# nexoedge/nexoedge

Measured on AMD Instinct MI355X. Metric: GiB/s RS(10,4) encode+decode, 1 MiB chunks, device-resident, higher is better.
Workload: dtype u8

## Files before the change

### nexoedge_amd/csrc/nxec_kernels.hip

```cpp
#include <hip/hip_runtime.h>

#include <algorithm>
#include <array>
#include <atomic>
#include <cstdio>
#include <cstdlib>
#include <cstring>
#include <utility>

#include "nxec_device.h"
#include "nxec_internal.h"
#include "nxec_scrub_rule.h"

namespace nxec {

namespace {

constexpr int kBlock = 1024;
constexpr int kMaxTemplK = 20;
constexpr int kLdsBytes = 160 * 1024;
constexpr int kPrefetchMaxK = 10;
constexpr int kPrefetchMaxKCopy = 8;
constexpr int kPermPrefetchMaxK = 4;
constexpr int kPermMaxK = 13;
// ... 122 lines not shown
template <int KD, int ROWS, int R>
struct ScrubBody {
  static constexpr int K = KD + ROWS;
  static constexpr int kLds = table_bytes(KD, R);
  static __device__ __forceinline__ void setup(const MulArgs &a, uint32_t *tab) {
    build_tables<R>(a.coef, KD, ROWS, tab);
  }
  const char *tlane;
  int32_t *status;
  __device__ ScrubBody(const uint32_t *tab, int32_t *st)
      : tlane(reinterpret_cast<const char *>(tab) + (threadIdx.x % R) * 4), status(st) {}
  __device__ __forceinline__ void operator()(const MulArgs &, uint32_t s, uint32_t, const u32x4 (&d)[K]) const {
    uint32_t acc[16];
    lookup_sources<KD, R>(tlane, d, acc);
    uint32_t o[4][4];
    rows_of(acc, o);
    uint32_t bad = 0;
#pragma unroll
    for (int r = 0; r < ROWS; r++)
      bad |= (o[r][0] ^ d[KD + r].x) | (o[r][1] ^ d[KD + r].y) | (o[r][2] ^ d[KD + r].z) | (o[r][3] ^ d[KD + r].w);
    const uint64_t hit = __ballot(bad != 0);
    if (hit != 0) {
      if (static_cast<int>(__lane_id()) == __ffsll(static_cast<unsigned long long>(hit)) - 1) scrub_flag(status, s);
    }
  }
};

__device__ __forceinline__ uint32_t perm_mul(const uint32_t *t, uint32_t nl, uint32_t nh, uint32_t ml, uint32_t mh) {
  const uint32_t l0 = __builtin_amdgcn_perm(t[1], t[0], nl), l1 = __builtin_amdgcn_perm(t[3], t[2], nl);
  const uint32_t h0 = __builtin_amdgcn_perm(t[5], t[4], nh), h1 = __builtin_amdgcn_perm(t[7], t[6], nh);
  return ((ml & l1) | (~ml & l0)) ^ ((mh & h1) | (~mh & h0));
}

template <int K, bool GATHER, bool COPY>
struct PermBody {
  static constexpr int kLds = K * 32;
  static __device__ __forceinline__ void setup(const MulArgs &a, uint32_t *tab) {
    uint8_t *tb = reinterpret_cast<uint8_t *>(tab);
    for (int i = threadIdx.x; i < K * 16; i += blockDim.x) {
      const int j = i >> 4, n = i & 15;
      const uint32_t c = a.coef[j];
      tb[32 * j + n] = static_cast<uint8_t>(gf_mul_dev(c, n));
      tb[32 * j + 16 + n] = static_cast<uint8_t>(gf_mul_dev(c, n << 4));
    }
  }
  const uint32_t *tab;
  __device__ explicit PermBody(const uint32_t *t) : tab(t) {}
  __device__ __forceinline__ void operator()(const MulArgs &a, uint32_t s, uint32_t vg, const u32x4 (&d)[K]) const {
    uint32_t z;
    asm volatile("s_mov_b32 %0, 0" : "=s"(z));
    const uint32_t *tt = tab + z;
    uint32_t o[4] = {0, 0, 0, 0};
#pragma unroll
    for (int j = 0; j < K; j++) {
      const uint32_t w[4] = {d[j].x, d[j].y, d[j].z, d[j].w};
#pragma unroll
      for (int q = 0; q < 4; q++) {
        const uint32_t x = w[q], x4 = x << 4;
        const uint32_t nl = x & 0x07070707u, nh = (x >> 4) & 0x07070707u;
        const uint32_t ml = __builtin_amdgcn_perm(x4, x4 << 8, 0x0B090A08u);
        const uint32_t mh = __builtin_amdgcn_perm(x, x << 8, 0x0B090A08u);
        o[q] ^= perm_mul(tt + 8 * j, nl, nh, ml, mh);
      }
    }
    st_stream(dst_row<GATHER>(a, s, 0) + static_cast<size_t>(vg) * 16, u32x4{o[0], o[1], o[2], o[3]});
    copy_through<K, COPY>(a, s, vg, d);
  }
};

__device__ uint32_t g_tile_queue[kQueueSlots * 32];

__device__ __forceinline__ uint32_t grab_async(uint32_t *q) {
  uint32_t g;
  asm volatile("global_atomic_add %0, %1, %2, off sc0" : "=&v"(g) : "v"(q), "v"(1u) : "memory");
  return g;
}
template <int N, int OFF>
__device__ __forceinline__ void publish(uint32_t ring_base, uint32_t g) {
  static_assert(N >= 0 && N < 64, "vmcnt is 6 bits");
  asm volatile("s_waitcnt vmcnt(%2)\n\tds_write_b32 %0, %1 offset:%3" ::"v"(ring_base), "v"(g), "n"(N), "n"(OFF)
               : "memory");
}

template <int K, bool PF, bool Q, bool QWAIT_K, class LoadF, class RunF>
__device__ __forceinline__ void tile_loop(const LoadF &load, const RunF &run, uint32_t ntiles, int32_t slot_arg,
                                          uint32_t T, uint32_t *ring) {
  if (Q && slot_arg >= 0) {
    uint32_t *q = g_tile_queue + static_cast<size_t>(slot_arg) * 32;
    if (threadIdx.x == 0) {
      ring[2] = atomicAdd(q, 1u);
      ring[3] = atomicAdd(q, 1u);
    }
    __syncthreads();
    auto run_start = [&](uint32_t r) -> uint32_t { return r * T; };
    uint32_t t = run_start(__builtin_amdgcn_readfirstlane(ring[2]));
    uint32_t nrun = run_start(__builtin_amdgcn_readfirstlane(ring[3]));
    uint32_t rend = t + T < ntiles ? t + T : ntiles;
    int slot = 0;
    uint32_t ring_base = static_cast<uint32_t>(reinterpret_cast<uintptr_t>(ring));
    asm volatile("" : "+v"(ring_base));
    auto ring_barrier = [] {
      __builtin_amdgcn_fence(__ATOMIC_RELEASE, "workgroup", "local");
      __builtin_amdgcn_s_barrier();
      __builtin_amdgcn_fence(__ATOMIC_ACQUIRE, "workgroup", "local");
    };
    auto step = [&](u32x4(&cur)[K], u32x4(&nxt)[K], bool pf) {
      const bool edge = t + 1 >= rend;
      const uint32_t tn = edge ? nrun : t + 1;
      uint32_t g = 0;
      if (edge && threadIdx.x == 0) g = grab_async(q);
      if (pf) {
        load(tn < ntiles ? tn : t, nxt);
        __builtin_amdgcn_sched_barrier(0);
      } else {
        load(t, cur);
        __builtin_amdgcn_sched_barrier(0);
      }
      run(t, cur);
      if (edge) {
        if (threadIdx.x == 0) {
          if (slot == 0) publish<QWAIT_K ? K : 0, 0>(ring_base, g);
          else publish<QWAIT_K ? K : 0, 4>(ring_base, g);
        }
        ring_barrier();
        const uint32_t nn = run_start(__builtin_amdgcn_readfirstlane(ring[slot]));
        slot ^= 1;
        rend = nrun + T < ntiles ? nrun + T : ntiles;
        nrun = nn;
      }
      t = tn;
      return t < ntiles;
    };
    if (t < ntiles) {
      if constexpr (PF) {
        u32x4 A[K], B[K];
        load(t, A);
        while (step(A, B, true) && step(B, A, true)) {
        }
      } else {
        bool more = true;
        while (more) {
          u32x4 d[K];
          more = step(d, d, false);
        }
      }
    }
    if (threadIdx.x == 0) {
      __threadfence();
      if (atomicAdd(q + 1, 1u) == gridDim.x - 1) {
        atomicExch(q, 0u);
        atomicExch(q + 1, 0u);
      }
    }
    return;
  }
  uint32_t t = __builtin_amdgcn_readfirstlane(
      static_cast<uint32_t>((static_cast<uint64_t>(blockIdx.x) * ntiles) / gridDim.x));
  const uint32_t tend = __builtin_amdgcn_readfirstlane(
      static_cast<uint32_t>((static_cast<uint64_t>(blockIdx.x + 1) * ntiles) / gridDim.x));
  if (t >= tend) return;
  if constexpr (PF) {
    u32x4 A[K], B[K];
    load(t, A);
    while (true) {
      const uint32_t tb = t + 1;
      load(tb < tend ? tb : t, B);
      __builtin_amdgcn_sched_barrier(0);
      run(t, A);
      if (tb >= tend) break;
      t = tb;
      const uint32_t ta = t + 1;
      load(ta < tend ? ta : t, A);
      __builtin_amdgcn_sched_barrier(0);
      run(t, B);
      if (ta >= tend) break;
      t = ta;
    }
  } else {
    for (; t < tend; t++) {
      u32x4 d[K];
      load(t, d);
      run(t, d);
    }
  }
}

template <int K, bool GATHER, bool FULL, bool PF, bool Q, class Body>
__device__ __forceinline__ void mul_tiles(const MulArgs &a, const Body &body, uint32_t *ring) {
  const uint32_t nvec = static_cast<uint32_t>(a.vec_count);
  const uint32_t tps = (nvec + kBlock - 1) / kBlock;
  const uint32_t ntiles = tps * static_cast<uint32_t>(a.nstripes);
  const uint32_t sg = a.stripe_group, ns = static_cast<uint32_t>(a.nstripes);
  auto load = [&](uint32_t t, u32x4(&d)[K]) { load_tile<K, GATHER, FULL>(a, tile_pos(t, tps, sg, ns), nvec, d); };
  auto run = [&](uint32_t t, const u32x4(&d)[K]) {
    const TilePos p = tile_pos(t, tps, sg, ns);
    if (FULL || p.v < nvec) body(a, p.s, static_cast<uint32_t>(a.vec_begin) + p.v, d);
  };
  tile_loop<K, PF, Q, FULL>(load, run, ntiles, a.queue_slot, a.tiles_per_grab, ring);
}

template <int K, int R, bool GATHER, bool COPY, bool FULL>
__global__ __launch_bounds__(kBlock) void k_mul_vec(const MulArgs a) {
  constexpr bool PF = vec_prefetch(K, COPY, FULL);
  constexpr bool Q = vec_queued(K, R);
  using Body = LdsBody<K, R, GATHER, COPY>;
  static_assert(Body::kLds + (Q ? kRingBytes : 0) == vec_lds(K, R), "tables, then the ring: what the launch asks for");
  extern __shared__ uint32_t tab[];
  Body::setup(a, tab);
  __syncthreads();
  mul_tiles<K, GATHER, FULL, PF, Q>(a, Body(tab), tab + Body::kLds / 4);
}

template <int K, bool GATHER, bool COPY, bool FULL>
__global__ __launch_bounds__(kBlock) void k_mul_perm(const MulArgs a) {
  constexpr bool PF = perm_prefetch(K);
  using Body = PermBody<K, GATHER, COPY>;
  static_assert(Body::kLds + kRingBytes == perm_lds(K), "tables, then the ring: what the launch asks for");
  extern __shared__ uint32_t tab[];
  Body::setup(a, tab);
  __syncthreads();
  mul_tiles<K, GATHER, FULL, PF, true>(a, Body(tab), tab + Body::kLds / 4);
}

struct RaggedArgs {
  const ListStripe *__restrict__ stripes;
  const uint32_t *__restrict__ tile_stripe;
  const uint32_t *__restrict__ stripe_tile0;
  uint32_t ntiles;
  int32_t k, rows, row0, queue_slot;
  uint32_t tiles_per_grab;
  uint8_t coef[kMaxRowsPerPass * (NXEC_MAX_K + 1)];
};

template <int K, int R>
__global__ __launch_bounds__(kBlock) void k_mul_ragged(const RaggedArgs a) {
  constexpr bool PF = ragged_prefetch(K);
  constexpr int kLds = table_bytes(K, R);
  static_assert(R == default_r(K) && kLds + kRingBytes == ragged_lds(K), "ragged kernels are queue-driven");
  extern __shared__ uint32_t tab[];
  build_tables<R>(a.coef, K, a.rows, tab);
  __syncthreads();
  const char *tl = reinterpret_cast<const char *>(tab) + (threadIdx.x % R) * 4;
  auto where = [&](uint32_t t, ListStripe &st, uint32_t &v) {
    const uint32_t s = a.tile_stripe[t];
    st = a.stripes[s];
    v = (t - a.stripe_tile0[s]) * kBlock + threadIdx.x;
  };
  auto load = [&](uint32_t t, u32x4(&d)[K]) {
    ListStripe st;
    uint32_t v;
    where(t, st, v);
    if (v * int64_t(16) < st.len) {
#pragma unroll
      for (int j = 0; j < K; j++) d[j] = ld_stream(st.src + j * st.src_cs + static_cast<size_t>(v) * 16);
    }
  };
  auto run = [&](uint32_t t, const u32x4(&d)[K]) {
    ListStripe st;
    uint32_t v;
    where(t, st, v);
    if (v * int64_t(16) < st.len) {
      uint32_t acc[16];
      lookup_sources<K, R>(tl, d, acc);
      uint8_t *row0 = st.dst + a.row0 * st.dst_cs;
      const int rows = a.rows;
      store_rows(acc, rows, [=](int r) { return row0 + r * st.dst_cs + static_cast<size_t>(v) * 16; });
    }
  };
  tile_loop<K, PF, true, true>(load, run, a.ntiles, a.queue_slot, a.tiles_per_grab, tab + kLds / 4);
}

struct MixedArgs {
  uint8_t *base;
  int64_t stripe_stride;
  const MixedSeg *__restrict__ segs;
  const uint32_t *__restrict__ order;
  const uint32_t *__restrict__ seg_of;
  uint32_t ntiles, tps, nvec;
  int32_t queue_slot;
  uint32_t tiles_per_grab;
};

constexpr int mixed_lds(int k) { return vec_lds(k, default_r(k)); }

template <class T>
__device__ __forceinline__ const __attribute__((address_space(4))) T *const_table(const T *p) {
  return (const __attribute__((address_space(4))) T *)(reinterpret_cast<uintptr_t>(p));
}

template <int K, int R>
__global__ __launch_bounds__(kBlock) void k_mul_mixed(const MixedArgs a) {
  constexpr bool PF = ragged_prefetch(K);
  constexpr int kLds = table_bytes(K, R);
  static_assert(R == default_r(K) && kLds + kRingBytes == mixed_lds(K), "mixed kernels are queue-driven");
  extern __shared__ uint32_t tab[];
  const char *tl = reinterpret_cast<const char *>(tab) + (threadIdx.x % R) * 4;
  uint32_t resident = ~0u;
  struct Where {
    uint32_t s, g, v;
  };
  auto where = [&](uint32_t t) -> Where {
    const uint32_t i = t / a.tps;
    return {static_cast<uint32_t>(__builtin_amdgcn_readfirstlane(const_table(a.order)[i])),
            static_cast<uint32_t>(__builtin_amdgcn_readfirstlane(const_table(a.seg_of)[i])),
            (t - i * a.tps) * kBlock + threadIdx.x};
  };
  auto load = [&](uint32_t t, u32x4(&d)[K]) {
    const Where w = where(t);
    if (w.v < a.nvec) {
      const auto *sg = const_table(a.segs) + w.g;
      const uint8_t *sb = a.base + static_cast<int64_t>(w.s) * a.stripe_stride;
      const uint32_t vo = w.v * 16u;
#pragma unroll
      for (int j = 0; j < K; j++) d[j] = ld_stream(sb + sg->src_off[j] + vo);
    }
  };
  auto run = [&](uint32_t t, const u32x4(&d)[K]) {
    const Where w = where(t);
    const auto *sg = const_table(a.segs) + w.g;
    const int rows = static_cast<int>(sg->rows);
    if (w.g != resident) {
      __builtin_amdgcn_fence(__ATOMIC_RELEASE, "workgroup", "local");
      __builtin_amdgcn_s_barrier();
      build_tables<R>(a.segs[w.g].coef, K, rows, tab);
      __builtin_amdgcn_fence(__ATOMIC_RELEASE, "workgroup", "local");
      __builtin_amdgcn_s_barrier();
      __builtin_amdgcn_fence(__ATOMIC_ACQUIRE, "workgroup", "local");
      resident = w.g;
    }
    if (w.v < a.nvec) {
      uint32_t acc[16];
      lookup_sources<K, R>(tl, d, acc);
      uint8_t *db = a.base + static_cast<int64_t>(w.s) * a.stripe_stride;
      const uint32_t vo = w.v * 16u;
      const uint32_t o0 = sg->dst_off[0], o1 = sg->dst_off[1], o2 = sg->dst_off[2], o3 = sg->dst_off[3];
      store_rows(acc, rows, [=](int r) { return db + (r == 0 ? o0 : r == 1 ? o1 : r == 2 ? o2 : o3) + vo; });
    }
  };
  tile_loop<K, PF, true, true>(load, run, a.ntiles, a.queue_slot, a.tiles_per_grab, tab + kLds / 4);
}

struct DecodeMixedArgs {
  const uint8_t *__restrict__ src;
  uint8_t *__restrict__ dst;
  int64_t src_stripe_stride, dst_stripe_stride;
  const DecodeSeg *__restrict__ segs;
  const uint32_t *__restrict__ order;
  const uint32_t *__restrict__ seg_of;
  uint32_t ntiles, tps, nvec;
  int32_t queue_slot;
  uint32_t tiles_per_grab;
};

constexpr int decode_mixed_lds(int k) { return vec_lds(k, default_r(k)); }

template <int K, int R>
__global__ __launch_bounds__(kBlock) void k_decode_mixed(const DecodeMixedArgs a) {
  constexpr bool PF = ragged_prefetch(K);
  constexpr int kLds = table_bytes(K, R);
  static_assert(K <= kMaxDecodeMixedK && R == default_r(K) && kLds + kRingBytes == decode_mixed_lds(K),
                "decode kernels are queue-driven");
  extern __shared__ uint32_t tab[];
  const char *tl = reinterpret_cast<const char *>(tab) + (threadIdx.x % R) * 4;
  uint32_t resident = ~0u;
  struct Where {
    uint32_t s, g, v;
  };
  auto where = [&](uint32_t t) -> Where {
    const uint32_t i = t / a.tps;
    return {static_cast<uint32_t>(__builtin_amdgcn_readfirstlane(const_table(a.order)[i])),
            static_cast<uint32_t>(__builtin_amdgcn_readfirstlane(const_table(a.seg_of)[i])),
            (t - i * a.tps) * kBlock + threadIdx.x};
  };
  auto load = [&](uint32_t t, u32x4(&d)[K]) {
    const Where w = where(t);
    if (w.v < a.nvec) {
      const auto *sg = const_table(a.segs) + w.g;
      const uint8_t *sb = a.src + static_cast<int64_t>(w.s) * a.src_stripe_stride;
      const uint32_t vo = w.v * 16u;
#pragma unroll
      for (int j = 0; j < K; j++) d[j] = ld_stream(sb + sg->src_off[j] + vo);
    }
  };
  auto run = [&](uint32_t t, const u32x4(&d)[K]) {
    const Where w = where(t);
    const auto *sg = const_table(a.segs) + w.g;
    const int rows = static_cast<int>(sg->rows);
    if (rows > 0 && w.g != resident) {
      __builtin_amdgcn_fence(__ATOMIC_RELEASE, "workgroup", "local");
      __builtin_amdgcn_s_barrier();
      build_tables<R>(a.segs[w.g].coef, K, rows, tab);
      __builtin_amdgcn_fence(__ATOMIC_RELEASE, "workgroup", "local");
      __builtin_amdgcn_s_barrier();
      __builtin_amdgcn_fence(__ATOMIC_ACQUIRE, "workgroup", "local");
      resident = w.g;
    }
    if (w.v < a.nvec) {
      uint8_t *db = a.dst + static_cast<int64_t>(w.s) * a.dst_stripe_stride;
      const uint32_t vo = w.v * 16u;
      if (rows > 0) {
        uint32_t acc[16];
        lookup_sources<K, R>(tl, d, acc);
        const uint32_t o0 = sg->dst_off[0], o1 = sg->dst_off[1], o2 = sg->dst_off[2], o3 = sg->dst_off[3];
        store_rows(acc, rows, [=](int r) { return db + (r == 0 ? o0 : r == 1 ? o1 : r == 2 ? o2 : o3) + vo; });
      }
#pragma unroll
      for (int j = 0; j < K; j++) {
        const uint32_t c = sg->copy_off[j];
        if (c != kNoCopy) st_stream(db + c + vo, d[j]);
      }
    }
  };
  tile_loop<K, PF, true, true>(load, run, a.ntiles, a.queue_slot, a.tiles_per_grab, tab + kLds / 4);
}

struct UpdateArgs {
  uint8_t *base;
  const UpdateItem *__restrict__ items;
  const uint32_t *__restrict__ tile_item;
  const int64_t *__restrict__ byte_prefix;
  int64_t nitems, nbytes;
  uint32_t ntiles;
  int32_t k, rows, last, queue_slot;
  uint32_t tiles_per_grab;
  uint32_t chunk_stride;
  uint32_t par_off[kMaxRowsPerPass];
  uint8_t coef[kMaxRowsPerPass * (NXEC_MAX_K + 1)];
};

constexpr int update_lds(int k) { return vec_lds(k, default_r(k)); }
constexpr int kUpdateSrc = 2 + kMaxRowsPerPass;
static_assert(kUpdateTileVecs == kBlock, "the planner's tiles are one vector per thread");

template <int R>
__global__ __launch_bounds__(kBlock) void k_update_vec(const UpdateArgs a) {
  constexpr int K = kUpdateSrc;
  extern __shared__ uint32_t tab[];
  build_tables<R>(a.coef, a.k, a.rows, tab);
  __syncthreads();
  const char *tl = reinterpret_cast<const char *>(tab) + (threadIdx.x % R) * 4;
  struct Where {
    const uint8_t *nw;
    uint8_t *sb;
    uint32_t col, chunk, count, v;
  };
  auto where = [&](uint32_t t) -> Where {
    const uint32_t i = __builtin_amdgcn_readfirstlane(const_table(a.tile_item)[t]);
    const auto *it = const_table(a.items) + i;
    return {it->d_new,
            a.base + it->stripe_off,
            static_cast<uint32_t>(__builtin_amdgcn_readfirstlane(it->col)),
            static_cast<uint32_t>(__builtin_amdgcn_readfirstlane(it->chunk)),
            static_cast<uint32_t>(__builtin_amdgcn_readfirstlane(it->count)),
            (t - static_cast<uint32_t>(__builtin_amdgcn_readfirstlane(it->first))) * kBlock + threadIdx.x};
  };
  auto load = [&](uint32_t t, u32x4(&d)[K]) {
    const Where w = where(t);
    if (w.v < w.count) {
      const uint32_t vo = w.col + w.v * 16u;
      d[0] = ld_stream(w.sb + w.chunk * a.chunk_stride + vo);
      d[1] = ld_stream(w.nw + w.v * 16u);
#pragma unroll
      for (int r = 0; r < kMaxRowsPerPass; r++)
        if (r < a.rows) d[2 + r] = ld_stream(w.sb + a.par_off[r] + vo);
    }
  };
  auto run = [&](uint32_t t, const u32x4(&d)[K]) {
    const Where w = where(t);
    if (w.v < w.count) {
      uint32_t acc[16];
#pragma unroll
      for (int i = 0; i < 16; i++) acc[i] = 0;
      lookup16<R>(tl + w.chunk * table_bytes(1, R), d[0] ^ d[1], acc);
      uint32_t o[4][4];
      rows_of(acc, o);
      const uint32_t vo = w.col + w.v * 16u;
#pragma unroll
      for (int r = 0; r < kMaxRowsPerPass; r++)
        if (r < a.rows)
          st_stream(w.sb + a.par_off[r] + vo, d[2 + r] ^ u32x4{o[r][0], o[r][1], o[r][2], o[r][3]});
      if (a.last) st_stream(w.sb + w.chunk * a.chunk_stride + vo, d[1]);
    }
  };
  tile_loop<K, true, true, false>(load, run, a.ntiles, a.queue_slot, a.tiles_per_grab,
                                  tab + table_bytes(a.k, R) / 4);
}

__global__ __launch_bounds__(256) void k_update_bytes(const UpdateArgs a) {
  extern __shared__ uint32_t tab[];
  const int k = a.k;
  build_tables<1>(a.coef, k, a.rows, tab);
  __syncthreads();
  for (int64_t i = blockIdx.x * static_cast<int64_t>(blockDim.x) + threadIdx.x; i < a.nbytes;
       i += static_cast<int64_t>(gridDim.x) * blockDim.x) {
    int64_t lo = 0, hi = a.nitems - 1;
    while (lo < hi) {
      const int64_t mid = (lo + hi + 1) >> 1;
      if (a.byte_prefix[mid] <= i) lo = mid;
      else hi = mid - 1;
    }
    const UpdateItem it = a.items[lo];
    const int64_t b = i - a.byte_prefix[lo];
    uint8_t *stripe = a.base + it.stripe_off;
    const int64_t c = static_cast<int64_t>(it.col) + b;
    uint8_t *data = stripe + static_cast<int64_t>(it.chunk) * a.chunk_stride + c;
    const uint8_t nw = it.d_new[b];
    const uint32_t e = tab[it.chunk * 256 + (*data ^ nw)];
    for (int r = 0; r < a.rows; r++) stripe[a.par_off[r] + c] ^= static_cast<uint8_t>(e >> (8 * r));
    if (a.last) *data = nw;
  }
}

template <bool GATHER>
__global__ __launch_bounds__(kBlock) void k_mul_vec_dyn(const MulArgs a) {
  extern __shared__ uint32_t tab[];
  const int k = a.k;
  build_tables<1>(a, k, tab);
  __syncthreads();
  const uint32_t nvec = static_cast<uint32_t>(a.vec_count);
  const uint32_t tps = (nvec + kBlock - 1) / kBlock;
  const uint32_t ntiles = tps * static_cast<uint32_t>(a.nstripes);
  const char *tl = reinterpret_cast<const char *>(tab);
  const uint32_t t0 = static_cast<uint32_t>((static_cast<uint64_t>(blockIdx.x) * ntiles) / gridDim.x);
  const uint32_t t1 = static_cast<uint32_t>((static_cast<uint64_t>(blockIdx.x + 1) * ntiles) / gridDim.x);
  for (uint32_t t = t0; t < t1; t++) {
    const uint32_t s = t / tps;
    const uint32_t vl = (t - s * tps) * kBlock + threadIdx.x;
    if (vl >= nvec) continue;
    const uint32_t v = static_cast<uint32_t>(a.vec_begin) + vl;
    uint32_t acc[16];
#pragma unroll
    for (int i = 0; i < 16; i++) acc[i] = 0;
    for (int j0 = 0; j0 < k; j0 += 4) {
      u32x4 d[4];
#pragma unroll
      for (int jj = 0; jj < 4; jj++)
        if (j0 + jj < k) d[jj] = ld_stream(src_chunk<GATHER>(a, s, j0 + jj) + static_cast<size_t>(v) * 16);
#pragma unroll
      for (int jj = 0; jj < 4; jj++) {
        if (j0 + jj < k) {
          lookup16<1>(tl + (j0 + jj) * 1024, d[jj], acc);
          const uint32_t c = a.copy_off[j0 + jj];
          if (!GATHER && a.any_copy && c != kNoCopy)
            st_stream(a.dst + static_cast<int64_t>(s) * a.dst_stripe_stride + c + static_cast<size_t>(v) * 16, d[jj]);
        }
      }
    }
    store_rows<GATHER>(a, s, v, acc);
  }
}

template <bool GATHER>
__global__ __launch_bounds__(256) void k_mul_bytes(const MulArgs a) {
  extern __shared__ uint32_t tab[];
  const int k = a.k;
  build_tables<1>(a, k, tab);
  __syncthreads();
  const int64_t span = a.len - a.byte_begin;
  const int64_t total = span * a.nstripes;
  for (int64_t i = blockIdx.x * static_cast<int64_t>(blockDim.x) + threadIdx.x; i < total;
       i += static_cast<int64_t>(gridDim.x) * blockDim.x) {
    const uint32_t s = static_cast<uint32_t>(i / span);
    const int64_t pos = a.byte_begin + (i - static_cast<int64_t>(s) * span);
    uint32_t acc = 0;
    for (int j = 0; j < k; j++) {
      const uint8_t x = src_chunk<GATHER>(a, s, j)[pos];
      acc ^= tab[j * 256 + x];
      const uint32_t c = a.copy_off[j];
      if (!GATHER && a.any_copy && c != kNoCopy) a.dst[static_cast<int64_t>(s) * a.dst_stripe_stride + c + pos] = x;
    }
    for (int r = 0; r < a.rows; r++) dst_row<GATHER>(a, s, r)[pos] = static_cast<uint8_t>(acc >> (8 * r));
  }
}

template <int KD, int ROWS, bool FULL>
__global__ __launch_bounds__(kBlock) void k_scrub_vec(const ScrubArgs a) {
  constexpr int K = KD + ROWS;
  constexpr int R = default_r(KD);
  constexpr bool PF = scrub_prefetch(K, FULL);
  using Body = ScrubBody<KD, ROWS, R>;
  static_assert(K <= kScrubMaxSrc && Body::kLds + kRingBytes == scrub_vec_lds(KD), "scrub kernels are queue-driven");
  extern __shared__ uint32_t tab[];
  Body::setup(a.m, tab);
  __syncthreads();
  mul_tiles<K, false, FULL, PF, true>(a.m, Body(tab, a.status), tab + Body::kLds / 4);
}

__global__ __launch_bounds__(256) void k_scrub_bytes(const ScrubArgs a) {
  extern __shared__ uint32_t tab[];
  const MulArgs &m = a.m;
  const int k = m.k;
  build_tables<1>(m, k, tab);
  __syncthreads();
  const int64_t span = m.len - m.byte_begin;
  const int64_t total = span * m.nstripes;
  for (int64_t i = blockIdx.x * static_cast<int64_t>(blockDim.x) + threadIdx.x; i < total;
       i += static_cast<int64_t>(gridDim.x) * blockDim.x) {
    const uint32_t s = static_cast<uint32_t>(i / span);
    const int64_t pos = m.byte_begin + (i - static_cast<int64_t>(s) * span);
    uint32_t acc = 0;
    for (int j = 0; j < k; j++) acc ^= tab[j * 256 + src_chunk<false>(m, s, j)[pos]];
    const uint8_t *stripe = m.src + static_cast<int64_t>(s) * m.src_stripe_stride;
    uint32_t par = 0;
    for (int r = 0; r < m.rows; r++) par |= static_cast<uint32_t>(stripe[a.par_off[r] + pos]) << (8 * r);
    if (acc != par) scrub_flag(a.status, s);
  }
}

__global__ __launch_bounds__(256) void k_scrub_locate(const ScrubLocateArgs a) {
  extern __shared__ uint32_t scrub_lds[];
  __shared__ int s_lo, s_hi;
  const int64_t s = blockIdx.x;
  if (a.status[s] == scrub::kClean) return;
  const int tid = threadIdx.x;
  if (tid == 0 && a.nbad) atomicAdd(a.nbad, 1ull);
  const int n = a.n, k = a.k, m = n - k;
  if (!(a.flags & NXEC_SCRUB_LOCATE) || m < 2) return;
  uint8_t *coef = reinterpret_cast<uint8_t *>(scrub_lds);
  uint8_t *syn = coef + (m * k + 15) / 16 * 16 + tid;
  for (int i = tid; i < m * k; i += 256) coef[i] = a.coef[i];
  if (tid == 0) {
    s_lo = INT32_MAX;
    s_hi = INT32_MIN;
  }
  __syncthreads();
  uint8_t *base = a.base + s * a.stripe_stride;
  const int64_t cs = a.chunk_stride;
  int32_t mine = scrub::kClean;
  for (int64_t i = tid; i < a.len; i += 256) {
    for (int r = 0; r < m; r++) syn[r * 256] = base[(k + r) * cs + i];
    for (int j = 0; j < k; j++) {
      const uint32_t x = base[j * cs + i];
      for (int r = 0; r < m; r++) syn[r * 256] ^= static_cast<uint8_t>(gf_mul_dev(coef[r * k + j], x));
    }
    uint8_t e;
    const int32_t c = scrub::locate(n, k, coef, [&](int r) { return syn[r * 256]; }, &e);
    if (c != scrub::kClean) mine = (mine == scrub::kClean || mine == c) ? c : scrub::kUnlocated;
  }
  if (mine != scrub::kClean) {
    atomicMin(&s_lo, mine);
    atomicMax(&s_hi, mine);
  }
  __syncthreads();
  const int32_t located = (s_lo == s_hi && s_lo >= 0) ? s_lo : scrub::kUnlocated;
  if (tid == 0) a.status[s] = located;
  if (!(a.flags & NXEC_SCRUB_REPAIR) || located < 0) return;
  if (located >= k) {
    const uint8_t *row = coef + (located - k) * k;
    uint8_t *p = base + located * cs;
    for (int64_t i = tid; i < a.len; i += 256) {
      uint32_t v = 0;
      for (int j = 0; j < k; j++) v ^= gf_mul_dev(row[j], base[j * cs + i]);
      if (p[i] != static_cast<uint8_t>(v)) p[i] = static_cast<uint8_t>(v);
    }
  } else {
    const uint32_t ic = scrub::inv(coef[located]);
    uint8_t *d = base + located * cs;
    for (int64_t i = tid; i < a.len; i += 256) {
      uint32_t s0 = base[k * cs + i];
      for (int j = 0; j < k; j++) s0 ^= gf_mul_dev(coef[j], base[j * cs + i]);
      if (s0) d[i] ^= static_cast<uint8_t>(gf_mul_dev(s0, ic));
    }
  }
}

struct ListArgs {
  const ListStripe *stripes;
  const int64_t *prefix;
// ... 340 lines not shown
  static const std::vector<KernelLds> list = [] {
    std::vector<KernelLds> l;
    list_kernels(l);
    list_encode_md5_kernels(l);
    list_files_md5_kernels(l);
    return l;
  }();
  return list;
}

int raise_lds(const void *fn, int bytes, const char *family, bool no_static) {
  hipFuncAttributes fa{};
  if (no_static && (hipFuncGetAttributes(&fa, fn) != hipSuccess || fa.sharedSizeBytes != 0))
    return set_error(NXEC_ERR_HIP, "%s: static LDS present (the tables must start at LDS byte 0)", family);
  const hipError_t e = hipFuncSetAttribute(fn, hipFuncAttributeMaxDynamicSharedMemorySize, bytes);
  if (e != hipSuccess) return set_error(NXEC_ERR_HIP, "hipFuncSetAttribute(%s): %s", family, hipGetErrorString(e));
  return NXEC_OK;
}

int prepare_kernels() {
  for (const KernelLds &e : kernel_lds_list())
    if (int rc = raise_lds(e.fn, e.bytes, e.family, e.no_static)) return rc;
  return NXEC_OK;
}

namespace {

uint32_t tiles_per_grab(int k, int rows, int copies) {
  const int units = k + rows + copies;
  return static_cast<uint32_t>(std::max(1, std::min(8, (12 + units - 1) / units)));
}

uint32_t stripe_group_for(int64_t vec_count, bool aliased) {
  return ((vec_count + kBlock - 1) / kBlock >= 128 && aliased) ? 8 : 1;
}

std::atomic<uint32_t> g_next_slot{0};

int reset_queue_slots(int first, int count, hipStream_t st) {
  void *base = nullptr;
  hipError_t e = hipGetSymbolAddress(&base, HIP_SYMBOL(g_tile_queue));
  if (e == hipSuccess) {
    if (count <= 0) {
      first = 0;
      count = kQueueSlots;
    }
    e = hipMemsetAsync(static_cast<uint8_t *>(base) + static_cast<size_t>(first) * 128, 0,
                       static_cast<size_t>(count) * 128, st);
  }
  return e == hipSuccess ? NXEC_OK : hip_fail(e, "tile-queue reset");
}

int launch_failed(hipError_t e, const char *family, int slot, hipStream_t st) {
  const int rc = set_error(NXEC_ERR_HIP, "launch %s: %s", family, hipGetErrorString(e));
  if (slot >= 0) (void)reset_queue_slots(slot, 1, st);
  return rc;
}

struct QueueLaunch {
  const char *family, *kkey;
  int k, rows, r;
  int gather, copy, full;
  int pf, q;
  uint32_t tpg, sg;
  int64_t grid;
  int lds;
  int32_t slot;
  const char *tail = nullptr;
};

void record_launch(const QueueLaunch &l) {
  char s[224];
  const size_t cap = sizeof s;
  int n = std::snprintf(s, cap, "family=%s %s=%d rows=%d r=%d", l.family, l.kkey, l.k, l.rows, l.r);
  if (l.gather >= 0) n += std::snprintf(s + n, cap - n, " gather=%d copy=%d", l.gather, l.copy);
  if (l.full >= 0) n += std::snprintf(s + n, cap - n, " full=%d", l.full);
  n += std::snprintf(s + n, cap - n, " pf=%d q=%d tpg=%u", l.pf, l.q, l.tpg);
  if (l.sg) n += std::snprintf(s + n, cap - n, " sg=%u", l.sg);
  n += std::snprintf(s + n, cap - n, " grid=%lld slot=%d", static_cast<long long>(l.grid), l.slot);
  if (l.tail) std::snprintf(s + n, cap - n, " %s", l.tail);
  launch_log_append("%s", s);
}

template <class Args>
int queue_launch(void (*fn)(Args), const Args &a, int32_t &slot, QueueLaunch &l, hipStream_t st, bool draw = true) {
  slot = l.slot = draw ? static_cast<int32_t>(g_next_slot.fetch_add(1, std::memory_order_relaxed) % kQueueSlots) : -1;
  if (launch_log_on()) record_launch(l);
  hipLaunchKernelGGL(fn, dim3(static_cast<unsigned>(l.grid)), dim3(kBlock), l.lds, st, a);
  const hipError_t e = hipGetLastError();
  return e == hipSuccess ? NXEC_OK : launch_failed(e, l.family, slot, st);
}

template <class F>
int split_vectors(int64_t vec_count, int64_t nstripes, const F &launch) {
  const int64_t tps = (vec_count + kBlock - 1) / kBlock;
  if (tps * nstripes >= (int64_t(1) << 32) || vec_count >= (int64_t(1) << 32))
    return set_error(NXEC_ERR_INVALID, "batch too large for one launch (split nstripes)");
  const int64_t full = vec_count / kBlock * kBlock;
  int rc = full > 0 ? launch(int64_t(0), full, true) : NXEC_OK;
  if (rc == NXEC_OK && vec_count > full) rc = launch(full, vec_count - full, false);
  return rc;
}

}

int launch_mul(const MulArgs &a, bool vec_ok, int num_cus, void *stream) {
  hipStream_t st = static_cast<hipStream_t>(stream);
  if (a.nstripes <= 0 || a.len <= 0) return NXEC_OK;
  if (vec_ok && a.vec_count > 0) {
    const bool gather = a.src_ptrs != nullptr, copy = a.any_copy != 0;
    const bool dyn = a.k > kMaxTemplK;
    int copies = 0;
    for (int j = 0; copy && j < a.k; j++) copies += a.copy_off[j] != kNoCopy;
    const uint32_t tpg = tiles_per_grab(a.k, a.rows, copies);
    const bool aliased = gather || a.src_chunk_stride % (int64_t(1) << 20) == 0;
    const uint32_t sg = tuning().stripe_group > 0 ? static_cast<uint32_t>(tuning().stripe_group)
                                                  : stripe_group_for(a.vec_count, aliased);
    const int rc = split_vectors(a.vec_count, a.nstripes, [&](int64_t begin, int64_t count, bool full) {
      MulArgs b = a;
      b.tiles_per_grab = tpg;
      b.stripe_group = sg;
      b.vec_begin = a.vec_begin + begin;
      b.vec_count = count;
      const LaunchInfo li = plan_launch(b.k, b.rows, count, b.nstripes, num_cus, full, copy, gather);
      QueueLaunch l{li.perm ? "k_mul_perm" : dyn ? "k_mul_vec_dyn" : "k_mul_vec", "k", b.k, b.rows,
                    li.lds_copies, gather, copy, full,
                    li.perm ? perm_prefetch(b.k) : !dyn && vec_prefetch(b.k, copy, full),
                    li.perm || (!dyn && vec_queued(b.k, li.lds_copies)), dyn ? 0 : tpg, dyn ? 1 : sg, li.grid,
                    li.lds_bytes, 0};
      return queue_launch(mul_kernel(li, b.k, gather, copy, full), b, b.queue_slot, l, st,
                          !dyn && !tuning().static_order);
    });
    if (rc) return rc;
  }
  if (a.byte_begin < a.len) {
    const int64_t total = (a.len - a.byte_begin) * a.nstripes;
    int64_t blocks = (total + 255) / 256;
    if (blocks > static_cast<int64_t>(num_cus) * 8) blocks = static_cast<int64_t>(num_cus) * 8;
    KernelFn fn = a.src_ptrs ? &k_mul_bytes<true> : &k_mul_bytes<false>;
    if (launch_log_on())
      launch_log_append("family=k_mul_bytes k=%d rows=%d r=1 gather=%d copy=%d full=0 pf=0 q=0 tpg=0 sg=1 grid=%lld "
                        "byte_begin=%lld",
                        a.k, a.rows, a.src_ptrs != nullptr, a.any_copy != 0, static_cast<long long>(blocks),
                        static_cast<long long>(a.byte_begin));
    hipLaunchKernelGGL(fn, dim3(static_cast<unsigned>(blocks)), dim3(256), bytes_lds(a.k), st, a);
    hipError_t e = hipGetLastError();
    if (e != hipSuccess) return hip_fail(e, "launch k_mul_bytes");
  }
  return NXEC_OK;
}

bool scrub_vec_shape(int k, int rows) {
  return k >= 1 && k <= kScrubMaxK && rows >= 1 && rows <= kMaxRowsPerPass && k + rows <= kScrubMaxSrc;
}

int launch_scrub_detect(const ScrubArgs &a0, bool vec_ok, int num_cus, void *stream) {
  hipStream_t st = static_cast<hipStream_t>(stream);
  ScrubArgs a = a0;
  MulArgs &m = a.m;
  if (m.nstripes <= 0 || m.len <= 0 || m.rows <= 0) return NXEC_OK;
  const bool vec = vec_ok && scrub_vec_shape(m.k, m.rows);
  m.vec_begin = 0;
  m.vec_count = vec ? m.len / 16 : 0;
  m.byte_begin = m.vec_count * 16;
  if (m.vec_count > 0) {
    for (int r = 0; r < m.rows; r++) m.src_off[m.k + r] = a.par_off[r];
    m.tiles_per_grab = tiles_per_grab(m.k, m.rows, 0);
    m.stripe_group = stripe_group_for(m.vec_count, m.src_chunk_stride % (int64_t(1) << 20) == 0);
    const int rc = split_vectors(m.vec_count, m.nstripes, [&](int64_t begin, int64_t count, bool full) {
      ScrubArgs b = a;
      b.m.vec_begin = begin;
      b.m.vec_count = count;
      const int64_t ntiles = (count + kBlock - 1) / kBlock * m.nstripes;
      QueueLaunch l{"k_scrub_vec", "kd", m.k, m.rows, default_r(m.k), -1, -1, full,
                    scrub_prefetch(m.k + m.rows, full), 1, m.tiles_per_grab, m.stripe_group,
                    std::min<int64_t>(num_cus, ntiles), 0, 0};
      return queue_launch(scrub_kernel(m.k, m.rows, full, &l.lds), b, b.m.queue_slot, l, st);
    });
    if (rc) return rc;
  }
  if (m.byte_begin < m.len) {
    const int64_t total = (m.len - m.byte_begin) * m.nstripes;
    int64_t blocks = (total + 255) / 256;
    if (blocks > static_cast<int64_t>(num_cus) * 8) blocks = static_cast<int64_t>(num_cus) * 8;
    if (launch_log_on())
      launch_log_append("family=k_scrub_bytes kd=%d rows=%d grid=%lld byte_begin=%lld", m.k, m.rows,
                        static_cast<long long>(blocks), static_cast<long long>(m.byte_begin));
    hipLaunchKernelGGL(k_scrub_bytes, dim3(static_cast<unsigned>(blocks)), dim3(256), bytes_lds(m.k), st, a);
    hipError_t e = hipGetLastError();
    if (e != hipSuccess) return hip_fail(e, "launch k_scrub_bytes");
  }
  return NXEC_OK;
}

int launch_scrub_locate(const ScrubLocateArgs &a, void *stream) {
  if (a.nstripes <= 0) return NXEC_OK;
  if (a.nstripes >= (int64_t(1) << 31)) return set_error(NXEC_ERR_INVALID, "scrub: too many stripes for one launch");
  const int m = a.n - a.k;
  const size_t lds = static_cast<size_t>((m * a.k + 15) / 16 * 16) + static_cast<size_t>(m) * 256;
  hipLaunchKernelGGL(k_scrub_locate, dim3(static_cast<unsigned>(a.nstripes)), dim3(256), lds,
                     static_cast<hipStream_t>(stream), a);
  hipError_t e = hipGetLastError();
  return e == hipSuccess ? NXEC_OK : hip_fail(e, "launch k_scrub_locate");
}

int reset_work_queues(void *stream) {
  const int rc = reset_queue_slots(0, 0, static_cast<hipStream_t>(stream));
  if (rc) return rc;
  const hipError_t e = hipStreamSynchronize(static_cast<hipStream_t>(stream));
  return e == hipSuccess ? NXEC_OK : hip_fail(e, "tile-queue reset sync");
}

int debug_poison_next_queue_slot(uint32_t next_tile) {
  void *base = nullptr;
  hipError_t e = hipGetSymbolAddress(&base, HIP_SYMBOL(g_tile_queue));
  const uint32_t slot = g_next_slot.load() % kQueueSlots;
  if (e == hipSuccess)
    e = hipMemcpy(static_cast<uint8_t *>(base) + static_cast<size_t>(slot) * 128, &next_tile, sizeof(next_tile),
                  hipMemcpyHostToDevice);
  return e == hipSuccess ? NXEC_OK : hip_fail(e, "tile-queue poison");
}

int launch_mul_list(int rows, int k, const uint8_t *coeffs, const ListStripe *d_stripes, const int64_t *d_prefix,
                    int64_t nstripes, int64_t total_units, int num_cus, void *stream) {
  if (nstripes <= 0 || total_units <= 0 || rows <= 0) return NXEC_OK;
  if (k < 1 || k > NXEC_MAX_K) return set_error(NXEC_ERR_INVALID, "k=%d out of range", k);
  int64_t blocks = (total_units + 255) / 256;
  if (blocks > static_cast<int64_t>(num_cus) * 8) blocks = static_cast<int64_t>(num_cus) * 8;
  for (int r0 = 0; r0 < rows; r0 += kMaxRowsPerPass) {
    ListArgs a;
    std::memset(&a, 0, sizeof(a));
    a.stripes = d_stripes;
    a.prefix = d_prefix;
    a.nstripes = nstripes;
    a.total = total_units;
    a.k = k;
    a.rows = rows - r0 < kMaxRowsPerPass ? rows - r0 : kMaxRowsPerPass;
    a.row0 = r0;
    for (int r = 0; r < a.rows; r++)
      for (int j = 0; j < k; j++) a.coef[r * k + j] = coeffs[static_cast<size_t>(r0 + r) * k + j];
    if (launch_log_on())
      launch_log_append("family=k_mul_list k=%d rows=%d grid=%lld", k, a.rows, static_cast<long long>(blocks));
    hipLaunchKernelGGL(k_mul_list, dim3(static_cast<unsigned>(blocks)), dim3(256), bytes_lds(k),
                       static_cast<hipStream_t>(stream), a);
    hipError_t e = hipGetLastError();
    if (e != hipSuccess) return hip_fail(e, "launch k_mul_list");
  }
  return NXEC_OK;
}

int launch_mul_ragged(int rows, int k, const uint8_t *coeffs, const ListStripe *d_stripes, const uint32_t *d_tile_stripe,
                      const uint32_t *d_stripe_tile0, int64_t ntiles, int num_cus, void *stream) {
  if (ntiles <= 0 || rows <= 0) return NXEC_OK;
  if (k < 1 || k > kMaxRaggedK) return set_error(NXEC_ERR_INVALID, "ragged launch: k=%d unsupported", k);
  if (ntiles >= (int64_t(1) << 32)) return set_error(NXEC_ERR_INVALID, "ragged launch: too many tiles");
  const int64_t grid = std::min<int64_t>(num_cus, ntiles);
  for (int r0 = 0; r0 < rows; r0 += kMaxRowsPerPass) {
    RaggedArgs a;
    std::memset(&a, 0, sizeof(a));
    a.stripes = d_stripes;
    a.tile_stripe = d_tile_stripe;
    a.stripe_tile0 = d_stripe_tile0;
    a.ntiles = static_cast<uint32_t>(ntiles);
    a.k = k;
    a.rows = rows - r0 < kMaxRowsPerPass ? rows - r0 : kMaxRowsPerPass;
    a.row0 = r0;
    a.tiles_per_grab = tiles_per_grab(k, a.rows, 0);
    for (int r = 0; r < a.rows; r++)
      for (int j = 0; j < k; j++) a.coef[r * k + j] = coeffs[static_cast<size_t>(r0 + r) * k + j];
    QueueLaunch l{"k_mul_ragged", "k", k, a.rows, default_r(k), -1, -1, -1, ragged_prefetch(k), 1,
                  a.tiles_per_grab, 0, grid, ragged_lds(k), 0};
    if (int rc = queue_launch(kRagged[k - 1], a, a.queue_slot, l, static_cast<hipStream_t>(stream))) return rc;
  }
  return NXEC_OK;
}

int launch_mul_mixed(int k, uint8_t *base, int64_t stripe_stride, int64_t len, const MixedSeg *d_segs,
                     const uint32_t *d_order, const uint32_t *d_seg_of, int64_t nitems, int64_t nsegs, int64_t ncoded,
                     int num_cus, void *stream) {
  if (nitems <= 0 || len <= 0) return NXEC_OK;
  if (k < 1 || k > kMaxRaggedK) return set_error(NXEC_ERR_INVALID, "mixed launch: k=%d unsupported", k);
  const int64_t nvec = len / 16, tps = (nvec + kBlock - 1) / kBlock;
  if (len % 16 || nvec >= (int64_t(1) << 32) || tps * nitems >= (int64_t(1) << 32))
    return set_error(NXEC_ERR_INVALID, "mixed launch: too many tiles or a sub-16-byte tail");
  MixedArgs a{};
  a.base = base;
  a.stripe_stride = stripe_stride;
  a.segs = d_segs;
  a.order = d_order;
  a.seg_of = d_seg_of;
  a.tps = static_cast<uint32_t>(tps);
  a.nvec = static_cast<uint32_t>(nvec);
  a.ntiles = static_cast<uint32_t>(tps * nitems);
  a.tiles_per_grab = tiles_per_grab(k, kMaxRowsPerPass, 0);
  char tail[64];
  std::snprintf(tail, sizeof tail, "segs=%lld stripes=%lld", static_cast<long long>(nsegs),
                static_cast<long long>(ncoded));
  QueueLaunch l{"k_mul_mixed", "k", k, kMaxRowsPerPass, default_r(k), -1, -1, -1, ragged_prefetch(k), 1,
                a.tiles_per_grab, 0, std::min<int64_t>(num_cus, a.ntiles), mixed_lds(k), 0, tail};
  return queue_launch(kMixed[k - 1], a, a.queue_slot, l, static_cast<hipStream_t>(stream));
}

int launch_decode_mixed(int k, const uint8_t *src, int64_t stripe_stride, uint8_t *dst, int64_t out_stripe_stride,
                        int64_t len, const DecodeSeg *d_segs, const uint32_t *d_order, const uint32_t *d_seg_of,
                        int64_t nitems, int64_t nsegs, int64_t ndecoded, int num_cus, void *stream) {
  if (nitems <= 0 || len <= 0) return NXEC_OK;
  if (k < 1 || k > kMaxDecodeMixedK) return set_error(NXEC_ERR_INVALID, "mixed decode launch: k=%d unsupported", k);
  const int64_t nvec = len / 16, tps = (nvec + kBlock - 1) / kBlock;
  if (len % 16 || nvec >= (int64_t(1) << 32) || tps * nitems >= (int64_t(1) << 32))
    return set_error(NXEC_ERR_INVALID, "mixed decode launch: too many tiles or a sub-16-byte tail");
  DecodeMixedArgs a{};
  a.src = src;
  a.dst = dst;
  a.src_stripe_stride = stripe_stride;
  a.dst_stripe_stride = out_stripe_stride;
  a.segs = d_segs;
  a.order = d_order;
  a.seg_of = d_seg_of;
  a.tps = static_cast<uint32_t>(tps);
  a.nvec = static_cast<uint32_t>(nvec);
  a.ntiles = static_cast<uint32_t>(tps * nitems);
  a.tiles_per_grab = tiles_per_grab(k, 0, k);
  char tail[64];
  std::snprintf(tail, sizeof tail, "segs=%lld stripes=%lld", static_cast<long long>(nsegs),
                static_cast<long long>(ndecoded));
  QueueLaunch l{"k_decode_mixed", "k", k, kMaxRowsPerPass, default_r(k), -1, -1, -1, ragged_prefetch(k), 1,
                a.tiles_per_grab, 0, std::min<int64_t>(num_cus, a.ntiles), decode_mixed_lds(k), 0, tail};
  return queue_launch(kDecodeMixed[k - 1], a, a.queue_slot, l, static_cast<hipStream_t>(stream));
}

namespace {
void update_pass(UpdateArgs &a, int k, int rows, int row0, const uint8_t *coef, uint8_t *base, int64_t chunk_stride,
                 bool last) {
  a.base = base;
  a.k = k;
  a.rows = rows;
  a.last = last;
  a.chunk_stride = static_cast<uint32_t>(chunk_stride);
  for (int r = 0; r < rows; r++) {
    a.par_off[r] = static_cast<uint32_t>((k + row0 + r) * chunk_stride);
    for (int j = 0; j < k; j++) a.coef[r * k + j] = coef[static_cast<size_t>(r) * k + j];
  }
}
}

int launch_update_vec(int k, int rows, int row0, const uint8_t *coef, uint8_t *base, int64_t chunk_stride,
                      const UpdateItem *d_items, const uint32_t *d_tile_item, int64_t ntiles, bool last,
                      int64_t nupdates, int round, int pass, int num_cus, void *stream) {
  if (ntiles <= 0) return NXEC_OK;
  if (k < 1 || k > kMaxRaggedK || rows < 0 || rows > kMaxRowsPerPass)
    return set_error(NXEC_ERR_INVALID, "update launch: k=%d rows=%d unsupported", k, rows);
  if (ntiles >= (int64_t(1) << 32)) return set_error(NXEC_ERR_INVALID, "update launch: too many tiles");
  UpdateArgs a{};
  update_pass(a, k, rows, row0, coef, base, chunk_stride, last);
  a.items = d_items;
  a.tile_item = d_tile_item;
  a.ntiles = static_cast<uint32_t>(ntiles);
  a.tiles_per_grab = tiles_per_grab(2 + (last ? 1 : 0), 2 * rows, 0);
  char tail[96];
  std::snprintf(tail, sizeof tail, "tiles=%lld updates=%lld round=%d pass=%d last=%d", static_cast<long long>(ntiles),
                static_cast<long long>(nupdates), round, pass, last ? 1 : 0);
  QueueLaunch l{"k_update_vec", "k", k, rows, default_r(k), -1, -1, -1, 1, 1, a.tiles_per_grab, 0,
                std::min<int64_t>(num_cus, ntiles), update_lds(k), 0, tail};
  return queue_launch(update_fn(k), a, a.queue_slot, l, static_cast<hipStream_t>(stream));
}

int launch_update_bytes(int k, int rows, int row0, const uint8_t *coef, uint8_t *base, int64_t chunk_stride,
                        const UpdateItem *d_items, const int64_t *d_byte_prefix, int64_t nitems, int64_t nbytes,
                        bool last, int round, int pass, int num_cus, void *stream) {
  if (nitems <= 0 || nbytes <= 0) return NXEC_OK;
  if (k < 1 || k > NXEC_MAX_K || rows < 0 || rows > kMaxRowsPerPass)
    return set_error(NXEC_ERR_INVALID, "update launch: k=%d rows=%d unsupported", k, rows);
  UpdateArgs a{};
  update_pass(a, k, rows, row0, coef, base, chunk_stride, last);
  a.items = d_items;
  a.byte_prefix = d_byte_prefix;
  a.nitems = nitems;
  a.nbytes = nbytes;
  a.queue_slot = -1;
  const int64_t blocks = std::min<int64_t>((nbytes + 255) / 256, static_cast<int64_t>(num_cus) * 8);
  if (launch_log_on())
    launch_log_append("family=k_update_bytes k=%d rows=%d r=1 grid=%lld items=%lld round=%d pass=%d last=%d", k, rows,
                      static_cast<long long>(blocks), static_cast<long long>(nitems), round, pass, last ? 1 : 0);
  hipLaunchKernelGGL(k_update_bytes, dim3(static_cast<unsigned>(blocks)), dim3(256), bytes_lds(k),
                     static_cast<hipStream_t>(stream), a);
  const hipError_t e = hipGetLastError();
  return e == hipSuccess ? NXEC_OK : hip_fail(e, "launch k_update_bytes");
}

int launch_pad_chunks(const PadChunks *d_items, const uint32_t *d_bstart, int64_t nitems, int64_t nblocks,
                      void *stream) {
  if (nitems <= 0 || nblocks <= 0) return NXEC_OK;
  if (nblocks >= (int64_t(1) << 31)) return set_error(NXEC_ERR_INVALID, "pad-chunks launch too large");
  hipLaunchKernelGGL(k_pad_chunks, dim3(static_cast<unsigned>(nblocks)), dim3(256), 0, static_cast<hipStream_t>(stream),
                     d_items, d_bstart, nitems);
  hipError_t e = hipGetLastError();
  return e == hipSuccess ? NXEC_OK : hip_fail(e, "launch k_pad_chunks");
}

int launch_copy16(void *dst, const void *src, size_t bytes, int num_cus, void *stream) {
  if (bytes == 0) return NXEC_OK;
  if (bytes % 16 || (reinterpret_cast<uintptr_t>(dst) | reinterpret_cast<uintptr_t>(src)) & 15)
    return set_error(NXEC_ERR_INVALID, "copy16: unaligned");
  const int64_t n = static_cast<int64_t>(bytes / 16);
  const int64_t blocks = std::min<int64_t>((n + 255) / 256, static_cast<int64_t>(num_cus) * 4);
  hipLaunchKernelGGL(k_copy16, dim3(static_cast<unsigned>(blocks)), dim3(256), 0, static_cast<hipStream_t>(stream),
                     static_cast<u32x4 *>(dst), static_cast<const u32x4 *>(src), n);
  hipError_t e = hipGetLastError();
  return e == hipSuccess ? NXEC_OK : hip_fail(e, "launch k_copy16");
}

int launch_fill(void *d, size_t bytes, uint64_t seed, void *stream) {
  if (bytes == 0) return NXEC_OK;
  hipLaunchKernelGGL(k_fill, dim3(2048), dim3(256), 0, static_cast<hipStream_t>(stream), static_cast<uint8_t *>(d),
                     static_cast<int64_t>(bytes), seed);
  hipError_t e = hipGetLastError();
  return e == hipSuccess ? NXEC_OK : hip_fail(e, "launch k_fill");
}

int launch_checksum(const void *d, size_t bytes, uint64_t *d_out, void *stream) {
  hipLaunchKernelGGL(k_checksum, dim3(1024), dim3(256), 0, static_cast<hipStream_t>(stream),
                     static_cast<const uint8_t *>(d), static_cast<int64_t>(bytes),
                     reinterpret_cast<unsigned long long *>(d_out));
  hipError_t e = hipGetLastError();
  return e == hipSuccess ? NXEC_OK : hip_fail(e, "launch k_checksum");
}

}
```

Measured before the change: 5847.

## Overlap LDS table setup with first tile load; skip queue for small launches

New measurement: 5841. No clear change (-0.1%).

```diff
diff --git a/nexoedge_amd/csrc/nxec_kernels.hip b/nexoedge_amd/csrc/nxec_kernels.hip
--- a/nexoedge_amd/csrc/nxec_kernels.hip
+++ b/nexoedge_amd/csrc/nxec_kernels.hip
@@ -228,10 +228,20 @@
                : "memory");
 }
 
-template <int K, bool PF, bool Q, bool QWAIT_K, class LoadF, class RunF>
+__device__ __forceinline__ void lds_barrier() {
+  __builtin_amdgcn_fence(__ATOMIC_RELEASE, "workgroup", "local");
+  __builtin_amdgcn_s_barrier();
+  __builtin_amdgcn_fence(__ATOMIC_ACQUIRE, "workgroup", "local");
+}
+struct NoSetup {
+  __device__ __forceinline__ void operator()() const {}
+};
+
+template <int K, bool PF, bool Q, bool QWAIT_K, class LoadF, class RunF, class SetupF>
 __device__ __forceinline__ void tile_loop(const LoadF &load, const RunF &run, uint32_t ntiles, int32_t slot_arg,
-                                          uint32_t T, uint32_t *ring) {
+                                          uint32_t T, uint32_t *ring, const SetupF &setup) {
   if (Q && slot_arg >= 0) {
+    setup();
     uint32_t *q = g_tile_queue + static_cast<size_t>(slot_arg) * 32;
     if (threadIdx.x == 0) {
       ring[2] = atomicAdd(q, 1u);
@@ -308,6 +318,8 @@
   if constexpr (PF) {
     u32x4 A[K], B[K];
     load(t, A);
+    __builtin_amdgcn_sched_barrier(0);
+    setup();
     while (true) {
       const uint32_t tb = t + 1;
       load(tb < tend ? tb : t, B);
@@ -323,6 +335,7 @@
       t = ta;
     }
   } else {
+    setup();
     for (; t < tend; t++) {
       u32x4 d[K];
       load(t, d);
@@ -332,7 +345,7 @@
 }
 
 template <int K, bool GATHER, bool FULL, bool PF, bool Q, class Body>
-__device__ __forceinline__ void mul_tiles(const MulArgs &a, const Body &body, uint32_t *ring) {
+__device__ __forceinline__ void mul_tiles(const MulArgs &a, const Body &body, uint32_t *tab, uint32_t *ring) {
   const uint32_t nvec = static_cast<uint32_t>(a.vec_count);
   const uint32_t tps = (nvec + kBlock - 1) / kBlock;
   const uint32_t ntiles = tps * static_cast<uint32_t>(a.nstripes);
@@ -342,7 +355,11 @@
     const TilePos p = tile_pos(t, tps, sg, ns);
     if (FULL || p.v < nvec) body(a, p.s, static_cast<uint32_t>(a.vec_begin) + p.v, d);
   };
-  tile_loop<K, PF, Q, FULL>(load, run, ntiles, a.queue_slot, a.tiles_per_grab, ring);
+  auto setup = [&] {
+    Body::setup(a, tab);
+    lds_barrier();
+  };
+  tile_loop<K, PF, Q, FULL>(load, run, ntiles, a.queue_slot, a.tiles_per_grab, ring, setup);
 }
 
 template <int K, int R, bool GATHER, bool COPY, bool FULL>
@@ -352,9 +369,7 @@
   using Body = LdsBody<K, R, GATHER, COPY>;
   static_assert(Body::kLds + (Q ? kRingBytes : 0) == vec_lds(K, R), "tables, then the ring: what the launch asks for");
   extern __shared__ uint32_t tab[];
-  Body::setup(a, tab);
-  __syncthreads();
-  mul_tiles<K, GATHER, FULL, PF, Q>(a, Body(tab), tab + Body::kLds / 4);
+  mul_tiles<K, GATHER, FULL, PF, Q>(a, Body(tab), tab, tab + Body::kLds / 4);
 }
 
 template <int K, bool GATHER, bool COPY, bool FULL>
@@ -363,9 +378,7 @@
   using Body = PermBody<K, GATHER, COPY>;
   static_assert(Body::kLds + kRingBytes == perm_lds(K), "tables, then the ring: what the launch asks for");
   extern __shared__ uint32_t tab[];
-  Body::setup(a, tab);
-  __syncthreads();
-  mul_tiles<K, GATHER, FULL, PF, true>(a, Body(tab), tab + Body::kLds / 4);
+  mul_tiles<K, GATHER, FULL, PF, true>(a, Body(tab), tab, tab + Body::kLds / 4);
 }
 
 struct RaggedArgs {
@@ -384,8 +397,10 @@
   constexpr int kLds = table_bytes(K, R);
   static_assert(R == default_r(K) && kLds + kRingBytes == ragged_lds(K), "ragged kernels are queue-driven");
   extern __shared__ uint32_t tab[];
-  build_tables<R>(a.coef, K, a.rows, tab);
-  __syncthreads();
+  auto setup = [&] {
+    build_tables<R>(a.coef, K, a.rows, tab);
+    lds_barrier();
+  };
   const char *tl = reinterpret_cast<const char *>(tab) + (threadIdx.x % R) * 4;
   auto where = [&](uint32_t t, ListStripe &st, uint32_t &v) {
     const uint32_t s = a.tile_stripe[t];
@@ -413,7 +428,7 @@
       store_rows(acc, rows, [=](int r) { return row0 + r * st.dst_cs + static_cast<size_t>(v) * 16; });
     }
   };
-  tile_loop<K, PF, true, true>(load, run, a.ntiles, a.queue_slot, a.tiles_per_grab, tab + kLds / 4);
+  tile_loop<K, PF, true, true>(load, run, a.ntiles, a.queue_slot, a.tiles_per_grab, tab + kLds / 4, setup);
 }
 
 struct MixedArgs {
@@ -483,7 +498,7 @@
       store_rows(acc, rows, [=](int r) { return db + (r == 0 ? o0 : r == 1 ? o1 : r == 2 ? o2 : o3) + vo; });
     }
   };
-  tile_loop<K, PF, true, true>(load, run, a.ntiles, a.queue_slot, a.tiles_per_grab, tab + kLds / 4);
+  tile_loop<K, PF, true, true>(load, run, a.ntiles, a.queue_slot, a.tiles_per_grab, tab + kLds / 4, NoSetup{});
 }
 
 struct DecodeMixedArgs {
@@ -557,7 +572,7 @@
       }
     }
   };
-  tile_loop<K, PF, true, true>(load, run, a.ntiles, a.queue_slot, a.tiles_per_grab, tab + kLds / 4);
+  tile_loop<K, PF, true, true>(load, run, a.ntiles, a.queue_slot, a.tiles_per_grab, tab + kLds / 4, NoSetup{});
 }
 
 struct UpdateArgs {
@@ -582,8 +597,10 @@
 __global__ __launch_bounds__(kBlock) void k_update_vec(const UpdateArgs a) {
   constexpr int K = kUpdateSrc;
   extern __shared__ uint32_t tab[];
-  build_tables<R>(a.coef, a.k, a.rows, tab);
-  __syncthreads();
+  auto setup = [&] {
+    build_tables<R>(a.coef, a.k, a.rows, tab);
+    lds_barrier();
+  };
   const char *tl = reinterpret_cast<const char *>(tab) + (threadIdx.x % R) * 4;
   struct Where {
     const uint8_t *nw;
@@ -629,7 +646,7 @@
     }
   };
   tile_loop<K, true, true, false>(load, run, a.ntiles, a.queue_slot, a.tiles_per_grab,
-                                  tab + table_bytes(a.k, R) / 4);
+                                  tab + table_bytes(a.k, R) / 4, setup);
 }
 
 __global__ __launch_bounds__(256) void k_update_bytes(const UpdateArgs a) {
@@ -727,9 +744,7 @@
   using Body = ScrubBody<KD, ROWS, R>;
   static_assert(K <= kScrubMaxSrc && Body::kLds + kRingBytes == scrub_vec_lds(KD), "scrub kernels are queue-driven");
   extern __shared__ uint32_t tab[];
-  Body::setup(a.m, tab);
-  __syncthreads();
-  mul_tiles<K, false, FULL, PF, true>(a.m, Body(tab, a.status), tab + Body::kLds / 4);
+  mul_tiles<K, false, FULL, PF, true>(a.m, Body(tab, a.status), tab, tab + Body::kLds / 4);
 }
 
 __global__ __launch_bounds__(256) void k_scrub_bytes(const ScrubArgs a) {
@@ -1236,8 +1251,14 @@
   launch_log_append("%s", s);
 }
 
+bool small_launch(int64_t ntiles, const QueueLaunch &l) {
+  return ntiles <= l.grid * static_cast<int64_t>(std::max<uint32_t>(l.tpg, 1u));
+}
+
 template <class Args>
-int queue_launch(void (*fn)(Args), const Args &a, int32_t &slot, QueueLaunch &l, hipStream_t st, bool draw = true) {
+int queue_launch(void (*fn)(Args), const Args &a, int32_t &slot, QueueLaunch &l, hipStream_t st, int64_t ntiles,
+                 bool draw = true) {
+  if (small_launch(ntiles, l)) draw = false;
   slot = l.slot = draw ? static_cast<int32_t>(g_next_slot.fetch_add(1, std::memory_order_relaxed) % kQueueSlots) : -1;
   if (launch_log_on()) record_launch(l);
   hipLaunchKernelGGL(fn, dim3(static_cast<unsigned>(l.grid)), dim3(kBlock), l.lds, st, a);
@@ -1283,7 +1304,7 @@
                     li.perm || (!dyn && vec_queued(b.k, li.lds_copies)), dyn ? 0 : tpg, dyn ? 1 : sg, li.grid,
                     li.lds_bytes, 0};
       return queue_launch(mul_kernel(li, b.k, gather, copy, full), b, b.queue_slot, l, st,
-                          !dyn && !tuning().static_order);
+                          (count + kBlock - 1) / kBlock * b.nstripes, !dyn && !tuning().static_order);
     });
     if (rc) return rc;
   }
@@ -1329,7 +1350,7 @@
       QueueLaunch l{"k_scrub_vec", "kd", m.k, m.rows, default_r(m.k), -1, -1, full,
                     scrub_prefetch(m.k + m.rows, full), 1, m.tiles_per_grab, m.stripe_group,
                     std::min<int64_t>(num_cus, ntiles), 0, 0};
-      return queue_launch(scrub_kernel(m.k, m.rows, full, &l.lds), b, b.m.queue_slot, l, st);
+      return queue_launch(scrub_kernel(m.k, m.rows, full, &l.lds), b, b.m.queue_slot, l, st, ntiles);
     });
     if (rc) return rc;
   }
@@ -1424,7 +1445,7 @@
       for (int j = 0; j < k; j++) a.coef[r * k + j] = coeffs[static_cast<size_t>(r0 + r) * k + j];
     QueueLaunch l{"k_mul_ragged", "k", k, a.rows, default_r(k), -1, -1, -1, ragged_prefetch(k), 1,
                   a.tiles_per_grab, 0, grid, ragged_lds(k), 0};
-    if (int rc = queue_launch(kRagged[k - 1], a, a.queue_slot, l, static_cast<hipStream_t>(stream))) return rc;
+    if (int rc = queue_launch(kRagged[k - 1], a, a.queue_slot, l, static_cast<hipStream_t>(stream), ntiles)) return rc;
   }
   return NXEC_OK;
 }
@@ -1452,7 +1473,7 @@
                 static_cast<long long>(ncoded));
   QueueLaunch l{"k_mul_mixed", "k", k, kMaxRowsPerPass, default_r(k), -1, -1, -1, ragged_prefetch(k), 1,
                 a.tiles_per_grab, 0, std::min<int64_t>(num_cus, a.ntiles), mixed_lds(k), 0, tail};
-  return queue_launch(kMixed[k - 1], a, a.queue_slot, l, static_cast<hipStream_t>(stream));
+  return queue_launch(kMixed[k - 1], a, a.queue_slot, l, static_cast<hipStream_t>(stream), a.ntiles);
 }
 
 int launch_decode_mixed(int k, const uint8_t *src, int64_t stripe_stride, uint8_t *dst, int64_t out_stripe_stride,
@@ -1480,7 +1501,7 @@
                 static_cast<long long>(ndecoded));
   QueueLaunch l{"k_decode_mixed", "k", k, kMaxRowsPerPass, default_r(k), -1, -1, -1, ragged_prefetch(k), 1,
                 a.tiles_per_grab, 0, std::min<int64_t>(num_cus, a.ntiles), decode_mixed_lds(k), 0, tail};
-  return queue_launch(kDecodeMixed[k - 1], a, a.queue_slot, l, static_cast<hipStream_t>(stream));
+  return queue_launch(kDecodeMixed[k - 1], a, a.queue_slot, l, static_cast<hipStream_t>(stream), a.ntiles);
 }
 
 namespace {
@@ -1516,7 +1537,7 @@
                 static_cast<long long>(nupdates), round, pass, last ? 1 : 0);
   QueueLaunch l{"k_update_vec", "k", k, rows, default_r(k), -1, -1, -1, 1, 1, a.tiles_per_grab, 0,
                 std::min<int64_t>(num_cus, ntiles), update_lds(k), 0, tail};
-  return queue_launch(update_fn(k), a, a.queue_slot, l, static_cast<hipStream_t>(stream));
+  return queue_launch(update_fn(k), a, a.queue_slot, l, static_cast<hipStream_t>(stream), ntiles);
 }
 
 int launch_update_bytes(int k, int rows, int row0, const uint8_t *coef, uint8_t *base, int64_t chunk_stride,
```
